# espiriki/Garbage_Classification_RCA

Hardware: AMD Instinct MI355X
Metric: train samples/sec (image+text pairs), MM-RCA ViT-B16+DistilBERT (higher is better)
Workload: dtype bf16

## Files before the change

garbage_classification_rca_amd/csrc/gemm256.hip:

```cpp
#include "common.h"
#include "lds_asm.h"
#include <type_traits>
#include <mutex>

typedef __attribute__((ext_vector_type(4))) float f32x4;
typedef __attribute__((address_space(3))) void lds_void;
typedef const __attribute__((address_space(1))) void gbl_void;

#define HT_BYTES (128 * 64 * 2)
#define STAGE_BYTES (4 * HT_BYTES)
#define LDS256_BYTES (128 * (256 * 4 + 16))
#define SLOT_A0 0
#define SLOT_A1 1
#define SLOT_B0 2
#define SLOT_B1 3

__device__ __forceinline__ int krow_f2(int row) { return (row & 3) | (((row >> 3) & 1) << 2); }

__device__ __forceinline__ void stage_half(const bf16_t* src0, const bf16_t* src1, char* lds_piece0) {
  __builtin_amdgcn_global_load_lds((gbl_void*)src0, (lds_void*)(lds_piece0), 16, 0, 0);
  __builtin_amdgcn_global_load_lds((gbl_void*)src1, (lds_void*)(lds_piece0 + 1024), 16, 0, 0);
}

template <bool F4>
// ... 400 lines not shown
    for (int a = 0; a < 2; ++a)
#pragma unroll
      for (int b = 0; b < 2; ++b)
#pragma unroll
        for (int i = 0; i < 4; ++i)
#pragma unroll
          for (int j = 0; j < 2; ++j) acc[a][b][i][j] = (f32x4){0.f, 0.f, 0.f, 0.f};
    frag_bases();
    if (wr) BARRIER();
    __builtin_amdgcn_sched_barrier(0);
    const int ntv = (X3 && !F4) ? nseg * nt : tile_nk;
    if constexpr (F4) {
      if (ti + 1 < my_tiles) {
        for (int t = 0; t < ntv; ++t) K_TILE_G4(ISSUE_P, 1, 1, 1, 1, 8, 8, 10, 8);
      } else {
        for (int t = 0; t < ntv - 2; ++t) K_TILE_G4(ISSUE_P, 1, 1, 1, 1, 8, 8, 10, 8);
        K_TILE_G4(ISSUE_P, 1, 1, 0, 0, 8, 8, 8, 4);
        K_TILE_G4(ISSUE_P, 0, 0, 0, 0, 2, 0, 0, 0);
      }
    } else
    if (ti + 1 < my_tiles) {
      for (int t = 0; t < ntv; ++t) K_TILE_G(ISSUE_P, 1, 1, 1, 1, 8, 8, 10, 8);
    } else {
      for (int t = 0; t < ntv - 2; ++t) K_TILE_G(ISSUE_P, 1, 1, 1, 1, 8, 8, 10, 8);
      K_TILE_G(ISSUE_P, 1, 1, 0, 0, 8, 8, 8, 4);
      K_TILE_G(ISSUE_P, 0, 0, 0, 0, 2, 0, 0, 0);
    }
    if (!wr) BARRIER();
    __builtin_amdgcn_sched_barrier(0);

    if constexpr (!X3 || F4) {
      if (ti >= my_dp) {
        int lane_s = lane;
        asm volatile("" : "+v"(lane_s));
        float* const mine = sk_slab + ((int64_t)(unit_tile * sk_split + unit_part) * 65536 + wave * 8192 + lane_s * 4);
#pragma unroll
        for (int f = 0; f < 32; ++f)
          asm volatile("global_store_dwordx4 %0, %1, off sc1" :: "v"(mine + f * 256), "v"(acc[f >> 4][(f >> 3) & 1][(f >> 1) & 3][f & 1]) : "memory");
        asm volatile("s_waitcnt vmcnt(0)" ::: "memory");
        __syncthreads();
        volatile unsigned* const flag = reinterpret_cast<volatile unsigned*>(smem + EP_BASE);
        if (threadIdx.x == 0) {
          const unsigned arrived = __hip_atomic_fetch_add(sk_count + unit_tile, 1u, __ATOMIC_RELAXED, __HIP_MEMORY_SCOPE_AGENT);
          if (arrived == (unsigned)sk_split - 1u)
            __hip_atomic_store(sk_count + unit_tile, 0u, __ATOMIC_RELAXED, __HIP_MEMORY_SCOPE_AGENT);
          *flag = arrived;
        }
        __syncthreads();
        const bool last = *flag == (unsigned)sk_split - 1u;
        __syncthreads();
        if (!last) break;
        asm volatile("" : "+v"(lane_s));
        const float* const all = sk_slab + ((int64_t)(unit_tile * sk_split) * 65536 + wave * 8192 + lane_s * 4);
#define SK_LD16(R, SRC)                                                                                                       \
        asm volatile("global_load_dwordx4 %0, %16, off sc1\n\tglobal_load_dwordx4 %1, %16, off offset:1024 sc1\n\t"         \
                     "global_load_dwordx4 %2, %16, off offset:2048 sc1\n\tglobal_load_dwordx4 %3, %16, off offset:3072 sc1\n\t" \
                     "global_load_dwordx4 %4, %17, off sc1\n\tglobal_load_dwordx4 %5, %17, off offset:1024 sc1\n\t"         \
                     "global_load_dwordx4 %6, %17, off offset:2048 sc1\n\tglobal_load_dwordx4 %7, %17, off offset:3072 sc1\n\t" \
                     "global_load_dwordx4 %8, %18, off sc1\n\tglobal_load_dwordx4 %9, %18, off offset:1024 sc1\n\t"         \
                     "global_load_dwordx4 %10, %18, off offset:2048 sc1\n\tglobal_load_dwordx4 %11, %18, off offset:3072 sc1\n\t" \
                     "global_load_dwordx4 %12, %19, off sc1\n\tglobal_load_dwordx4 %13, %19, off offset:1024 sc1\n\t"       \
                     "global_load_dwordx4 %14, %19, off offset:2048 sc1\n\tglobal_load_dwordx4 %15, %19, off offset:3072 sc1\n\t" \
                     "s_waitcnt vmcnt(0)"                                                                                     \
                     : "=&v"(R[0]), "=&v"(R[1]), "=&v"(R[2]), "=&v"(R[3]), "=&v"(R[4]), "=&v"(R[5]), "=&v"(R[6]), "=&v"(R[7]),     \
                       "=&v"(R[8]), "=&v"(R[9]), "=&v"(R[10]), "=&v"(R[11]), "=&v"(R[12]), "=&v"(R[13]), "=&v"(R[14]), "=&v"(R[15]) \
                     : "v"((SRC)), "v"((SRC) + 1024), "v"((SRC) + 2048), "v"((SRC) + 3072) : "memory")
        for (int part = 0; part < sk_split; ++part) {
          const float* const src = all + (int64_t)part * 65536;
#pragma unroll
          for (int h = 0; h < 2; ++h) {
            f32x4 t[16];
            SK_LD16(t, src + h * 4096);
#pragma unroll
            for (int f = 0; f < 16; ++f) {
              f32x4& c = acc[h][(f >> 3) & 1][(f >> 1) & 3][f & 1];
              c = part == 0 ? t[f] : c + t[f];
            }
          }
        }
#undef SK_LD16
      }
    }

    int lane_e = lane;
    asm volatile("" : "+v"(lane_e));
    const int e16 = lane_e & 15, eg = lane_e >> 4;
    const unsigned wbase0 = lds0 + EP_BASE + wave * 4096 + e16 * 256 + ((eg ^ (e16 & 7)) << 4);
    const unsigned rbase0 = lds0 + EP_BASE + wave * 4096 + eg * 256;
    const int64_t ncol = n_blk + 64 * wc + 4 * e16;
    const unsigned lane_off = (unsigned)(eg * (int)ldc + 4 * e16) * 2u;
    float bv[4] = {0.f, 0.f, 0.f, 0.f};
    if constexpr (act != MMRCA_ACT_MUL) {
      if (bias) {
        if constexpr (X3) {
          const f32x4 b4 = *reinterpret_cast<const f32x4*>(reinterpret_cast<const float*>(bias) + ncol);
#pragma unroll
          for (int r = 0; r < 4; ++r) bv[r] = b4[r];
        } else {
          bf16x4 b4 = *reinterpret_cast<const bf16x4*>(bias + ncol);
#pragma unroll
          for (int r = 0; r < 4; ++r) bv[r] = (float)b4[r];
        }
      }
    }
    float csum[4] = {0.f, 0.f, 0.f, 0.f};
    const bool full = m_blk + 256 <= M;
    asm volatile("s_nop 15\n\ts_nop 15" ::: "memory");
    constexpr bool SIDE = ADD || act == MMRCA_ACT_MUL;
    bf16x4 side[SIDE ? 32 : 1];
    if constexpr (SIDE) {
      const char* sp = reinterpret_cast<const char*>(ADD ? (const bf16_t*)addend : (const bf16_t*)preact);
      if (!(dbg & 2)) {
#pragma unroll
        for (int q = 0; q < 32; ++q) {
          const int64_t urow = m_blk + 128 * (q >> 4) + 64 * wr + 4 * (q & 15);
          const int64_t ub = (urow * ldc + n_blk + 64 * wc) * 2;
          side[q] = *reinterpret_cast<const bf16x4*>(sp + ub + lane_off);
        }
      }
    }
    auto passes = [&](auto ragged_tag) {
      constexpr bool RAGGED = decltype(ragged_tag)::value;
  #pragma unroll
      for (int pass = 0; pass < 8; ++pass) {
        const int a = pass >> 2, i = pass & 3;
        {
          const unsigned wbase1 = wbase0 ^ 64u;
          DS_WRITE_B128(wbase0, acc[a][0][i][0], 0);
          DS_WRITE_B128(wbase1, acc[a][0][i][1], 0);
          DS_WRITE_B128(wbase0, acc[a][1][i][0], 128);
          DS_WRITE_B128(wbase1, acc[a][1][i][1], 128);
        }
        const int64_t urow0 = m_blk + 128 * a + 64 * wr + 16 * i;
        constexpr int RB = SIDE ? 2 : 4;
  #pragma unroll
        for (int it0 = 0; it0 < 4; it0 += RB) {
          f32x4 cr[RB];
  #pragma unroll
          for (int u = 0; u < RB; ++u) {
            const int it = it0 + u;
            const unsigned rb = rbase0 + it * 1024 + ((unsigned)(e16 ^ ((4 * it + eg) & 7)) << 4);
            DS_READ_B128(cr[u], rb, 0);
          }
          if constexpr (RB == 4) asm volatile("s_waitcnt lgkmcnt(0)" : "+v"(cr[0]), "+v"(cr[1]), "+v"(cr[2]), "+v"(cr[3]) :: "memory");
          else asm volatile("s_waitcnt lgkmcnt(0)" : "+v"(cr[0]), "+v"(cr[1]) :: "memory");
  #pragma unroll
          for (int u = 0; u < RB; ++u) {
            const int it = it0 + u;
            float v[4] = {cr[u][0], cr[u][1], cr[u][2], cr[u][3]};
            if constexpr (act != MMRCA_ACT_MUL) {
  #pragma unroll
              for (int r = 0; r < 4; ++r) v[r] += bv[r];
            }
            bf16x4 po;
            [[maybe_unused]] float pf[4] = {0.f, 0.f, 0.f, 0.f};
            constexpr bool store_pre = act == MMRCA_ACT_GELU_SAVE_GRAD;
            if constexpr (act == MMRCA_ACT_MUL) {
  #pragma unroll
              for (int r = 0; r < 4; ++r) v[r] *= (float)side[4 * pass + it][r];
            } else if constexpr (act == MMRCA_ACT_GELU_SAVE_GRAD) {
              float gr[4];
              gelu_and_grad_fast4(v, gr);
  #pragma unroll
              for (int r = 0; r < 4; ++r) { po[r] = (bf16_t)gr[r]; pf[r] = gr[r]; }
            } else if constexpr (act == MMRCA_ACT_GELU) {
              gelu_fast4(v);
            }
            if constexpr (ADD) {
  #pragma unroll
              for (int r = 0; r < 4; ++r) v[r] += (float)side[4 * pass + it][r];
            }
            bf16x4 o;
  #pragma unroll
            for (int r = 0; r < 4; ++r) o[r] = (bf16_t)v[r];
            const bool ok = !RAGGED || urow0 + 4 * it + eg < M;
            if (ok) {
              if constexpr (act == MMRCA_ACT_MUL) {
  #pragma unroll
                for (int r = 0; r < 4; ++r) csum[r] += (float)o[r];
              }
              const int64_t ub = ((urow0 + 4 * it) * ldc + n_blk + 64 * wc) * 2;
              if constexpr (X3) {
                if (store_pre) {
                  if (pre16) *reinterpret_cast<bf16x4*>(reinterpret_cast<char*>(preact) + ub + lane_off) = po;
                  else *reinterpret_cast<f32x4*>(reinterpret_cast<char*>(preact) + 2 * (ub + lane_off)) = (f32x4){pf[0], pf[1], pf[2], pf[3]};
                }
                if constexpr (PLANES) {
                  bf16x4 lo;
#pragma unroll
                  for (int r = 0; r < 4; ++r) lo[r] = (bf16_t)(v[r] - (float)o[r]);
                  *reinterpret_cast<bf16x4*>(reinterpret_cast<char*>(C) + ub + lane_off) = o;
                  *reinterpret_cast<bf16x4*>(reinterpret_cast<char*>(C_lo) + ub + lane_off) = lo;
                } else {
                  *reinterpret_cast<f32x4*>(reinterpret_cast<char*>(C) + 2 * (ub + lane_off)) = (f32x4){v[0], v[1], v[2], v[3]};
                }
              } else {
              if (store_pre) *reinterpret_cast<bf16x4*>(reinterpret_cast<char*>(preact) + ub + lane_off) = po;
              *reinterpret_cast<bf16x4*>(reinterpret_cast<char*>(C) + ub + lane_off) = o;
              }
            }
          }
        }
      }
    };
    if (!(dbg & 2)) {
      if (full) passes(std::false_type{}); else passes(std::true_type{});
    }
    if constexpr (act == MMRCA_ACT_MUL) {
      if (colsum) {
#pragma unroll
        for (int r = 0; r < 4; ++r) atomicAdd(colsum + ncol + r, csum[r]);
      }
    }
    __builtin_amdgcn_sched_barrier(0);
  }
}

extern int g_mmrca_dbg;

#define SK_COUNTER_BYTES 4096
#define SK_MAX_UNITS 256
struct SkWorkspace { int device; void* stream; char* base; int64_t bytes; };
static SkWorkspace g_sk_ws[32];
static int g_sk_ws_n = 0;
static std::mutex g_sk_mutex;
extern "C" int64_t mmrca_gemm_streamk_workspace_bytes(void) { return SK_COUNTER_BYTES + (int64_t)SK_MAX_UNITS * 65536 * 4; }
extern "C" int mmrca_gemm_streamk_workspace(void* workspace, int64_t bytes, void* stream) {
  MMRCA_REQUIRE(workspace == nullptr || (bytes >= mmrca_gemm_streamk_workspace_bytes() && (((uintptr_t)workspace) & 15) == 0),
                "gemm_streamk_workspace: needs %lld bytes, 16-byte aligned, zero-filled", (long long)mmrca_gemm_streamk_workspace_bytes());
  int dev = 0;
  (void)hipGetDevice(&dev);
  std::lock_guard<std::mutex> lock(g_sk_mutex);
  for (int i = 0; i < g_sk_ws_n; ++i)
    if (g_sk_ws[i].stream == stream && g_sk_ws[i].device == dev) {
      if (workspace) { g_sk_ws[i].base = (char*)workspace; g_sk_ws[i].bytes = bytes; }
      else g_sk_ws[i] = g_sk_ws[--g_sk_ws_n];
      return 0;
    }
  if (!workspace || g_sk_ws_n == 32) return 0;
  g_sk_ws[g_sk_ws_n++] = SkWorkspace{dev, stream, (char*)workspace, bytes};
  return 0;
}
static char* sk_workspace_of(void* stream) {
  if (g_sk_ws_n == 0) return nullptr;
  int dev = 0;
  (void)hipGetDevice(&dev);
  std::lock_guard<std::mutex> lock(g_sk_mutex);
  for (int i = 0; i < g_sk_ws_n; ++i)
    if (g_sk_ws[i].stream == stream && g_sk_ws[i].device == dev) return g_sk_ws[i].base;
  return nullptr;
}
static int g_sk_max = 4, g_sk_min_ksteps = 24;
static bool g_sk_bf16 = false;
extern "C" int mmrca_gemm_streamk_config(int max_split, int min_ksteps, int bf16_products) {
  if (max_split >= 0) g_sk_max = max_split;
  if (min_ksteps >= 0) g_sk_min_ksteps = min_ksteps;
  if (bf16_products >= 0) g_sk_bf16 = bf16_products != 0;
  return 0;
}
int mmrca_gemm256_streamk_split(int64_t M, int64_t N, int64_t ksteps, void* stream, bool x3) {
  const int sk_max = g_sk_max;
  if ((!x3 && !g_sk_bf16) || ksteps < g_sk_min_ksteps || !sk_workspace_of(stream)) return 0;
  const int64_t tiles = ((M + 255) / 256) * (N / 256);
  const int ncu = cu_count();
  if (tiles < ncu) return 0;
  const int64_t left = tiles % ncu;
  if (left == 0) return 0;
  int64_t split = ncu / left;
  if (split > ksteps / 2) split = ksteps / 2;
  if (split > sk_max) split = sk_max;
  return split >= 2 ? (int)split : 0;
}
int64_t mmrca_gemm256_round_split(int64_t M, int64_t N) {
  const int64_t ncu = cu_count(), tm = M / 256, tn = N / 256, tiles = tm * tn;
  const int64_t rounds = tiles / ncu, rem = tiles - rounds * ncu;
  const int64_t m_split = rounds * ncu / tn;
  return rounds >= 1 && rem * 100 >= 25 * ncu && rem * 100 < 60 * ncu && m_split >= 1 && m_split < tm ? m_split * 256 : 0;
}
template <bool AK, bool BK2, int ACT, bool ADD, bool X3 = false, bool PLANES = false, bool F4 = false>
static void launch_p256(const void* A, const void* B, void* C, const void* bias, const void* addend, void* preact, int64_t M,
                        int64_t N, int64_t K, int64_t lda, int64_t ldb, int64_t ldc, float* colsum, hipStream_t st,
                        const void* A_lo = nullptr, const void* B_lo = nullptr, void* C_lo = nullptr, int nseg = 3, int pre16 = 0) {
  const int tiles_m = (int)((M + 255) / 256), tiles_n = (int)(N / 256);
  const int ncu = cu_count();
  int grid = tiles_m * tiles_n < ncu ? ((tiles_m * tiles_n) & ~7) : ncu;
  if (grid < 8) grid = 8;
  constexpr int LDS_P = 2 * STAGE_BYTES + 32768;
  int sk_split = 0;
  char* sk_ws = nullptr;
  if constexpr (!X3 || F4) {
    sk_split = mmrca_gemm256_streamk_split(M, N, K / (F4 ? 32 : 64), (void*)st, X3);
    if (sk_split >= 2) sk_ws = sk_workspace_of((void*)st);
    if (!sk_ws) sk_split = 0;
  }
  MMRCA_MAX_LDS(LDS_P, gemm_p256_k<AK, BK2, ACT, ADD, X3, PLANES, F4>);
  hipLaunchKernelGGL((gemm_p256_k<AK, BK2, ACT, ADD, X3, PLANES, F4>), dim3(grid), dim3(512), LDS_P, st, (const bf16_t*)A, (const bf16_t*)B,
                     (bf16_t*)C, (const bf16_t*)bias, (const bf16_t*)addend, (bf16_t*)preact, M, N, K, lda, ldb, ldc, tiles_m,
                     tiles_n, colsum, 0, g_mmrca_dbg, (const bf16_t*)A_lo,
                     (const bf16_t*)B_lo, (bf16_t*)C_lo, nseg, pre16, (float*)(sk_ws ? sk_ws + SK_COUNTER_BYTES : nullptr),
                     (unsigned*)sk_ws, sk_split);
}

int g_mmrca_dbg = 0;
extern "C" int mmrca_debug_set(int v) { g_mmrca_dbg = v; return 0; }

bool mmrca_gemm256_ok(int64_t M, int64_t N, int64_t K, int a_layout, int act, bool has_addend, bool has_preact, bool has_colsum, bool has_bias) {
  if (!(N % 256 == 0 && K % 64 == 0 && K >= 128 && a_layout == MMRCA_ROWK)) return false;
  if (act == MMRCA_ACT_NONE) return !has_preact && !has_colsum;
  if (act == MMRCA_ACT_GELU_SAVE_GRAD) return has_preact && !has_addend && !has_colsum;
  if (act == MMRCA_ACT_GELU) return !has_preact && !has_addend && !has_colsum;
  if (act == MMRCA_ACT_MUL) return has_preact && !has_addend && !has_bias;
  return false;
}

int mmrca_gemm256(const void* A, const void* B, void* C, const void* bias, const void* addend, void* preact, int64_t M,
                  int64_t N, int64_t K, int64_t lda, int64_t ldb, int64_t ldc, int a_layout, int b_layout, int act,
                  float* colsum, hipStream_t st) {
  const bool bk = b_layout == MMRCA_KROW;
  MMRCA_REQUIRE(mmrca_gemm256_ok(M, N, K, a_layout, act, addend != nullptr, preact != nullptr, colsum != nullptr, bias != nullptr),
                "gemm(mfma256): shape / epilogue combination not built");
  MMRCA_REQUIRE(M * lda * 2 < (1ll << 32) && (bk ? K * ldb : N * ldb) * 2 < (1ll << 32) && M * ldc * 2 < (1ll << 32),
                "gemm(mfma256): operands must be smaller than 4 GiB");
  with_bools([&](auto bk_) {
    const auto launch = [&](auto mode, auto add) {
      launch_p256<false, bk_, mode, add>(A, B, C, bias, addend, preact, M, N, K, lda, ldb, ldc, colsum, st);
    };
    using std::integral_constant;
    if (act == MMRCA_ACT_GELU_SAVE_GRAD) launch(integral_constant<int, MMRCA_ACT_GELU_SAVE_GRAD>{}, std::false_type{});
    else if (act == MMRCA_ACT_GELU) launch(integral_constant<int, MMRCA_ACT_GELU>{}, std::false_type{});
    else if (act == MMRCA_ACT_MUL) launch(integral_constant<int, MMRCA_ACT_MUL>{}, std::false_type{});
    else if (addend) launch(integral_constant<int, MMRCA_ACT_NONE>{}, std::true_type{});
    else launch(integral_constant<int, MMRCA_ACT_NONE>{}, std::false_type{});
  }, bk);
  MMRCA_CHECK_LAUNCH("gemm(mfma256)");
  return 0;
}


bool mmrca_gemm256_x3_ok(int64_t M, int64_t N, int64_t K, int a_layout, int act, bool has_addend, bool has_colsum) {
  if (!(N % 256 == 0 && K % 64 == 0 && K >= 128 && a_layout == MMRCA_ROWK) || has_addend || has_colsum) return false;
  return act == MMRCA_ACT_NONE || act == MMRCA_ACT_GELU_SAVE_GRAD;
}

int mmrca_gemm256_x3_streamk_split(int64_t M, int64_t N, int64_t K, int b_layout, bool has_a_lo, bool has_b_lo, void* stream) {
  if (!(b_layout != MMRCA_KROW && has_a_lo && has_b_lo && K % 32 == 0 && K >= 64)) return 0;
  return mmrca_gemm256_streamk_split(M, N, K / 32, stream, true);
}

int mmrca_gemm256_x3(const void* A_hi, const void* A_lo, const void* B_hi, const void* B_lo, void* C, void* C_lo, const void* bias,
                     void* preact, int64_t M, int64_t N, int64_t K, int64_t lda, int64_t ldb, int64_t ldc, int b_layout, int act,
                     hipStream_t st, int pre16) {
  const bool bk = b_layout == MMRCA_KROW;
  MMRCA_REQUIRE(M * lda * 2 < (1ll << 32) && (bk ? K * ldb : N * ldb) * 2 < (1ll << 32) && M * ldc * 4 < (1ll << 32),
                "gemm_x3(mfma256): operands must be smaller than 4 GiB");
  const bool gelu = act == MMRCA_ACT_GELU_SAVE_GRAD, planes = C_lo != nullptr;
  if (!bk && A_lo && B_lo && K % 32 == 0 && K >= 64) {
    with_bools([&](auto gelu_, auto planes_) {
      launch_p256<false, false, gelu_ ? MMRCA_ACT_GELU_SAVE_GRAD : MMRCA_ACT_NONE, false, true, planes_, true>(
          A_hi, B_hi, C, bias, nullptr, preact, M, N, K, lda, ldb, ldc, nullptr, st, A_lo, B_lo, C_lo, 3, pre16);
    }, gelu, planes);
    MMRCA_CHECK_LAUNCH("gemm_x3(mfma256,fused)");
    return 0;
  }
  with_bools([&](auto bk_, auto gelu_, auto planes_) {
    launch_p256<false, bk_, gelu_ ? MMRCA_ACT_GELU_SAVE_GRAD : MMRCA_ACT_NONE, false, true, planes_>(
        A_hi, B_hi, C, bias, nullptr, preact, M, N, K, lda, ldb, ldc, nullptr, st, A_lo, B_lo, C_lo, A_lo ? (B_lo ? 3 : 2) : 1, pre16);
  }, bk, gelu, planes);
  MMRCA_CHECK_LAUNCH("gemm_x3(mfma256)");
  return 0;
}

__global__ void __launch_bounds__(256)
splitk_reduce256_k(const float* __restrict__ slab, float* __restrict__ C, int64_t ldc, int ntiles, int tiles_n, int splits, int64_t M, int64_t N) {
  const int tile = blockIdx.x >> 6;
  const int idx = ((blockIdx.x & 63) << 8) + threadIdx.x;
  const float* src = slab + (int64_t)tile * 65536 + (int64_t)idx * 4;
  f32x4 s = *reinterpret_cast<const f32x4*>(src);
  for (int k = 1; k < splits; ++k) {
    const f32x4 v = *reinterpret_cast<const f32x4*>(src + (int64_t)k * ntiles * 65536);
    s += v;
  }
  const int w = idx >> 11, f = (idx >> 6) & 31, lane = idx & 63;
  const int a = f >> 4, b = (f >> 3) & 1, i = (f >> 1) & 3, j = f & 1;
  const int wr = w >> 2, wc = w & 3, l16 = lane & 15, g = lane >> 4;
  const int row = 128 * a + 64 * wr + 16 * i + l16, col = 128 * b + 32 * wc + 16 * j + 4 * g;
  const int tm = tile / tiles_n, tn = tile % tiles_n;
  if ((int64_t)tm * 256 + row >= M || (int64_t)tn * 256 + col >= N) return;
  float* dst = C + ((int64_t)tm * 256 + row) * ldc + (int64_t)tn * 256 + col;
  f32x4 c = *reinterpret_cast<f32x4*>(dst);
  c += s;
  *reinterpret_cast<f32x4*>(dst) = c;
}

extern "C" int64_t mmrca_gemm_splitk_workspace_bytes(int64_t M, int64_t N) {
  if (M <= 0 || N <= 0 || M % 8 || N % 8) return 0;
  const int64_t tiles = ((M + 255) / 256) * ((N + 255) / 256);
  if (tiles > 256) return 0;
  return (256 / tiles) * tiles * 65536 * 4;
}

static int gemm_splitk_impl(const void* A, const void* A_lo, const void* B, const void* B_lo, float* C, void* workspace,
                           int64_t workspace_bytes, int64_t M, int64_t N, int64_t K, int64_t lda, int64_t ldb, int64_t ldc,
                           int a_layout, int b_layout, void* stream) {
  const bool x3 = A_lo != nullptr;
  const int nseg = x3 ? (B_lo ? 3 : 2) : 1;
  MMRCA_REQUIRE(A && B && C && workspace, "gemm_splitk: null operand");
  const bool ragged = M % 256 != 0 || N % 256 != 0;
  MMRCA_REQUIRE(M > 0 && N > 0 && M % 8 == 0 && N % 8 == 0 && K >= 128 && K % 64 == 0 &&
                (!ragged || (a_layout == MMRCA_KROW && b_layout == MMRCA_KROW && !A_lo)),
                "gemm_splitk: needs K %% 64 == 0, K >= 128 and M, N multiples of 256 (K-major bf16 operands: of 8) (got M=%lld N=%lld K=%lld)",
                (long long)M, (long long)N, (long long)K);
  MMRCA_REQUIRE(lda % 8 == 0 && ldb % 8 == 0 && ldc % 4 == 0 && (((uintptr_t)A | (uintptr_t)B | (uintptr_t)C | (uintptr_t)workspace) & 15) == 0,
                "gemm_splitk: operands must be 16-byte aligned");
  MMRCA_REQUIRE(lda >= (a_layout == MMRCA_ROWK ? K : M) && ldb >= (b_layout == MMRCA_ROWK ? K : N) && ldc >= N, "gemm_splitk: leading dimension too small");
  const int tiles_m = (int)((M + 255) / 256), tiles_n = (int)((N + 255) / 256), tiles = tiles_m * tiles_n;
  MMRCA_REQUIRE(tiles <= 256, "gemm_splitk: more than 256 output tiles (use mmrca_gemm)");
  const int64_t ksteps = (int64_t)nseg * (K / 64);
  int64_t splits64 = 256 / tiles;
  if (splits64 > ksteps / 2) splits64 = ksteps / 2;
  const int splits = (int)splits64;
  const int ksteps_base = (int)(ksteps / splits), ksteps_rem = (int)(ksteps % splits);
  MMRCA_REQUIRE(workspace_bytes >= (int64_t)splits * tiles * 65536 * 4, "gemm_splitk: workspace too small (%lld < %lld bytes)",
                (long long)workspace_bytes, (long long)splits * tiles * 65536 * 4);
  hipStream_t st = (hipStream_t)stream;
  const bool ak = a_layout == MMRCA_KROW, bk = b_layout == MMRCA_KROW;
#define LSLAB(AK_, BK_, X3_)                                                                                                     \
  do {                                                                                                                           \
    MMRCA_MAX_LDS(LDS256_BYTES, gemm_mfma256_k<AK_, BK_, MODE_SLAB, X3_>); \
    hipLaunchKernelGGL((gemm_mfma256_k<AK_, BK_, MODE_SLAB, X3_>), dim3((tiles * splits + 7) / 8 * 8), dim3(512), LDS256_BYTES, st, (const bf16_t*)A,      \
                       (const bf16_t*)B, (bf16_t*)nullptr, (const bf16_t*)nullptr, (const bf16_t*)nullptr, (bf16_t*)nullptr, M, N, K, \
                       lda, ldb, ldc, tiles_m, tiles_n, ksteps_base, ksteps_rem, (float*)workspace, (float*)nullptr, splits,    \
                       (const bf16_t*)A_lo, (const bf16_t*)B_lo, nseg);                                                         \
  } while (0)
  if (x3) {
    if (!ak && !bk) LSLAB(false, false, true);
    else if (!ak && bk) LSLAB(false, true, true);
    else if (ak && !bk) LSLAB(true, false, true);
    else LSLAB(true, true, true);
  } else {
    if (!ak && !bk) LSLAB(false, false, false);
    else if (!ak && bk) LSLAB(false, true, false);
    else if (ak && !bk) LSLAB(true, false, false);
    else LSLAB(true, true, false);
  }
#undef LSLAB
  MMRCA_CHECK_LAUNCH("gemm_splitk(mfma256)");
  hipLaunchKernelGGL(splitk_reduce256_k, dim3(tiles * 64), dim3(256), 0, st, (const float*)workspace, C, ldc, tiles, tiles_n, splits, M, N);
  MMRCA_CHECK_LAUNCH("gemm_splitk(reduce)");
  return 0;
}

extern "C" int mmrca_gemm_splitk(const void* A, const void* B, float* C, void* workspace, int64_t workspace_bytes, int64_t M,
                                 int64_t N, int64_t K, int64_t lda, int64_t ldb, int64_t ldc, int a_layout, int b_layout,
                                 void* stream) {
  return gemm_splitk_impl(A, nullptr, B, nullptr, C, workspace, workspace_bytes, M, N, K, lda, ldb, ldc, a_layout, b_layout, stream);
}

extern "C" int mmrca_gemm_splitk_x3(const void* A_hi, const void* A_lo, const void* B_hi, const void* B_lo, float* C, void* workspace,
                                    int64_t workspace_bytes, int64_t M, int64_t N, int64_t K, int64_t lda, int64_t ldb, int64_t ldc,
                                    int a_layout, int b_layout, void* stream) {
  MMRCA_REQUIRE(A_lo || !B_lo, "gemm_x3(splitk): a B lo plane without an A lo plane is not a supported pass set");
  return gemm_splitk_impl(A_hi, A_lo, B_hi, B_lo, C, workspace, workspace_bytes, M, N, K, lda, ldb, ldc, a_layout, b_layout, stream);
}
```

garbage_classification_rca_amd/lib.py:

```python
from __future__ import annotations

import ctypes as C
import os
import subprocess
from types import SimpleNamespace
from typing import Optional

import torch

from . import abi

_HERE = os.path.dirname(os.path.abspath(__file__))
LIB_PATH = os.path.join(_HERE, "libmmrca.so")

F32, BF16 = 0, 1
ACT_NONE, ACT_GELU, ACT_GELU_BWD, ACT_GELU_SAVE_GRAD, ACT_MUL, ACT_GELU_SAVE_GRAD_BF16 = 0, 1, 2, 3, 4, 5
ROWK, KROW = 0, 1
IMPL_AUTO, IMPL_REF, IMPL_MFMA, IMPL_MFMA256, IMPL_MFMA_PERSIST, IMPL_MFMA_BK32, IMPL_MFMA_1STAGE, IMPL_MFMA_TALL, IMPL_MFMA_256W, IMPL_MFMA_256X4 = 0, 1, 2, 3, 4, 5, 6, 7, 8, 9

HEAD_FIELDS = [f"{blk}_{leaf}" for blk in ("sai", "sat", "c1", "c2")
               for leaf in ("wq", "bq", "wk", "bk", "wv", "bv", "g", "b")] + ["fin_w", "fin_b"]


class HeadPtrs(C.Structure):
    _fields_ = [(n, C.c_void_p) for n in HEAD_FIELDS]


class MmrcaError(RuntimeError):
    pass


def build_library(force: bool = False) -> str:
    src_dir = os.path.join(_HERE, "csrc")
    cmd = ["make", "-C", src_dir, "-j8"]
    if force:
        subprocess.run(["make", "-C", src_dir, "clean"], check=True, capture_output=True)
    r = subprocess.run(cmd, capture_output=True, text=True)
    if r.returncode != 0 or not os.path.exists(LIB_PATH) or not os.path.exists(os.path.join(_HERE, "libmmrca_jpeg.so")):
        raise MmrcaError("building libmmrca.so / libmmrca_jpeg.so failed:\n" + r.stdout[-4000:] + r.stderr[-4000:])
    return LIB_PATH


_lib = None
_protos = None


def _prototypes():
    global _protos
    if _protos is None:
        head = C.POINTER(HeadPtrs)
        try:
            _protos = abi.prototypes(struct_pointers={"MmrcaHeadWeights": head, "MmrcaHeadGrads": head})
        except abi.MmrcaError as e:
            raise MmrcaError(str(e)) from None
    return _protos


def load(build_if_missing: bool = False):
    global _lib
    if _lib is not None:
        return _lib
    if not os.path.exists(LIB_PATH):
        if build_if_missing:
            build_library()
        else:
            raise MmrcaError(f"{LIB_PATH} not found: the HIP extension is required (run __graft_entry__.build()); "
                             "there is no CPU fallback")
    lib = C.CDLL(LIB_PATH)
    try:
        abi.bind(lib, _prototypes())
    except abi.MmrcaError as e:
        raise MmrcaError(str(e)) from None
    _lib = lib
    return lib


def _check(rc: int, what: str):
    if rc != 0:
        raise MmrcaError(f"{what} failed ({rc}): {load().mmrca_last_error().decode()}")


def dtype_code(dt: torch.dtype) -> int:
    if dt == torch.float32:
        return F32
    if dt == torch.bfloat16:
        return BF16
    raise MmrcaError(f"unsupported dtype {dt}")


def ptr(t: Optional[torch.Tensor]):
    return None if t is None else t.data_ptr()


_raw_stream = getattr(torch._C, "_cuda_getCurrentRawStream", None)
_cur_device = getattr(torch._C, "_cuda_getDevice", None)


def stream_ptr() -> int:
    if _raw_stream is not None and _cur_device is not None:
        return _raw_stream(_cur_device())
    return torch.cuda.current_stream().cuda_stream


def _dev(t: torch.Tensor, name: str):
    if not t.is_cuda:
        raise MmrcaError(f"{name}: tensor must live in HBM (got device {t.device}); the product path has no CPU fallback")


def _launch(name, *args):
    rc = getattr(_lib if _lib is not None else load(), name)(*args, stream_ptr())
    if rc != 0:
        _check(rc, name)


GEMM_PROFILE = None
KERNEL_PROFILE = None


def _events():
    e0, e1 = torch.cuda.Event(enable_timing=True), torch.cuda.Event(enable_timing=True)
    e0.record()
    return e0, e1


class _Bracket:

    def __init__(self, kind, meta):
        self.kind, self.meta, self.on = kind, meta, KERNEL_PROFILE is not None

    def __enter__(self):
        if self.on:
            self.e0, self.e1 = _events()
        return self

    def __exit__(self, *exc):
        if self.on and exc[0] is None:
            self.e1.record()
            KERNEL_PROFILE.append((self.kind, self.meta, self.e0, self.e1))
        return False


def _esz(dt):
    return 2 if dt == BF16 else 4


GEMM_SHAPES = None
CONV_PROFILE = None


_STREAMK_WS = {}
STREAMK = os.environ.get("MMRCA_SK", "1") != "0"


def streamk_workspace(M, N, device, force=False):
    if not (STREAMK or force) or N % 256 or ((M + 255) // 256) * (N // 256) < 256:
        return
    st = stream_ptr()
    key = (device.index if device.index is not None else torch.cuda.current_device(), st)
    if key in _STREAMK_WS:
        return
    if not force and torch.cuda.is_current_stream_capturing():
        return
    need = int(load().mmrca_gemm_streamk_workspace_bytes())
    ws = torch.zeros(need, dtype=torch.uint8, device=device)
    _launch("mmrca_gemm_streamk_workspace", ptr(ws), need)
    _STREAMK_WS[key] = ws


def gemm_is_mfma(M, N, K, a_layout, dtype, impl):
    return dtype == BF16 and impl != IMPL_REF and N % 128 == 0 and K % 64 == 0 and (a_layout == ROWK or M % 128 == 0)


def gemm(A, B, Cout, *, bias=None, addend=None, preact=None, M, N, K, lda, ldb, ldc, a_layout=ROWK, b_layout=ROWK,
         act=ACT_NONE, accum=False, dtype, impl=IMPL_AUTO, colsum=None, rows_readable=None):
    _dev(A, "gemm A")
    if rows_readable is not None:
        if accum:
            raise MmrcaError("gemm: rows_readable is not available in accumulate mode")
        _launch("mmrca_gemm_rows", ptr(A), ptr(B), ptr(Cout), ptr(bias), ptr(addend), ptr(preact), ptr(colsum), M, N, K, lda, ldb, ldc,
                int(rows_readable[0]), int(rows_readable[1]), a_layout, b_layout, act, dtype, impl)
        return
    prof = GEMM_PROFILE is not None and (gemm_is_mfma(M, N, K, a_layout, dtype, impl) or (dtype == F32 and impl != IMPL_REF))
    timed = prof or CONV_PROFILE is not None
    if timed:
        e0, e1 = _events()
    if colsum is not None:
        if accum:
            raise MmrcaError("gemm: colsum is not available in accumulate mode")
        _launch("mmrca_gemm_colsum", ptr(A), ptr(B), ptr(Cout), ptr(bias), ptr(addend), ptr(preact), ptr(colsum), M, N, K, lda, ldb, ldc, a_layout,
                b_layout, act, dtype, impl)
    else:
        _launch("mmrca_gemm", ptr(A), ptr(B), ptr(Cout), ptr(bias), ptr(addend), ptr(preact), M, N, K, lda, ldb, ldc, a_layout, b_layout, act,
                int(accum), dtype, impl)
    if timed:
        e1.record()
    if prof:
        GEMM_PROFILE.append((2.0 * M * N * K, (a_layout, b_layout, int(accum)), e0, e1, (M, N, K, act)))
    if CONV_PROFILE is not None:
        es = _esz(dtype)
        side = (1 if addend is not None else 0) + (1 if preact is not None else 0)
        nbytes = int((M * K + N * K) * es + M * N * ((4 if accum else es) + side * es))
        CONV_PROFILE.append(("GEMM (1x1 conv / patch matrix / text encoder)", nbytes, e0, e1))
        if GEMM_SHAPES is not None:
            GEMM_SHAPES.append((M, N, K, a_layout, b_layout, int(accum), nbytes, e0, e1))


SPLITK_WS_BYTES = 64 << 20


def gemm_splitk_ok(M, N, K, dtype):
    return dtype == BF16 and M % 256 == 0 and N % 256 == 0 and K % 64 == 0 and K >= 128 and (M // 256) * (N // 256) <= 256


def gemm_splitk_ragged_ok(M, N, K, dtype):
    return (dtype == BF16 and M % 8 == 0 and N % 8 == 0 and K % 64 == 0 and K >= 128
            and ((M + 255) // 256) * ((N + 255) // 256) <= 256)


def gemm_splitk(A, B, Cout, workspace, *, M, N, K, lda, ldb, ldc, a_layout=KROW, b_layout=KROW):
    _dev(A, "gemm_splitk A")
    prof = GEMM_PROFILE is not None
    if prof:
        e0, e1 = _events()
    _launch("mmrca_gemm_splitk", ptr(A), ptr(B), ptr(Cout), ptr(workspace), workspace.numel() * workspace.element_size(), M, N, K, lda, ldb, ldc,
            a_layout, b_layout)
    if prof:
        e1.record()
        GEMM_PROFILE.append((2.0 * M * N * K, (a_layout, b_layout, 1), e0, e1, (M, N, K, ACT_NONE)))
    if CONV_PROFILE is not None:
        CONV_PROFILE.append(("GEMM (1x1 conv / patch matrix / text encoder)", int((M * K + N * K) * 2 + M * N * 4), None, None))


def gemm_x3(A, B, Cout, *, C_lo=None, bias=None, addend=None, preact=None, colsum=None, M, N, K, lda, ldb, ldc, a_layout=ROWK,
            b_layout=ROWK, act=ACT_NONE, accum=False, impl=IMPL_AUTO):
    _dev(A[0], "gemm_x3 A")
    if not accum:
        streamk_workspace(M, N, A[0].device)
    prof = GEMM_PROFILE is not None
    if prof:
        e0, e1 = _events()
    _launch("mmrca_gemm_x3", ptr(A[0]), ptr(A[1]), ptr(B[0]), ptr(B[1]), ptr(Cout), ptr(C_lo), ptr(bias), ptr(addend), ptr(preact), ptr(colsum), M, N,
            K, lda, ldb, ldc, a_layout, b_layout, act, int(accum), impl)
    if prof:
        e1.record()
        GEMM_PROFILE.append((6.0 * M * N * K, (a_layout, b_layout, int(accum)), e0, e1, (M, N, K, act)))


def gemm_splitk_x3(A, B, Cout, workspace, *, M, N, K, lda, ldb, ldc, a_layout=KROW, b_layout=KROW):
    _dev(A[0], "gemm_splitk_x3 A")
    prof = GEMM_PROFILE is not None
    if prof:
        e0, e1 = _events()
    _launch("mmrca_gemm_splitk_x3", ptr(A[0]), ptr(A[1]), ptr(B[0]), ptr(B[1]), ptr(Cout), ptr(workspace),
            workspace.numel() * workspace.element_size(), M, N, K, lda, ldb, ldc, a_layout, b_layout)
    if prof:
        e1.record()
        GEMM_PROFILE.append((6.0 * M * N * K, (a_layout, b_layout, 1), e0, e1, (M, N, K, ACT_NONE)))


def split_f32(src, hi, lo, n):
    _dev(src, "split src")
    _launch("mmrca_split_f32", ptr(src), ptr(hi), ptr(lo), n)


def colsum_accum(dY, db, M, N, ld, dtype):
    _launch("mmrca_colsum_accum", ptr(dY), ptr(db), M, N, ld, dtype)


def gelu_bwd(dG, H, dH, n, dtype):
    _launch("mmrca_gelu_bwd", ptr(dG), ptr(H), ptr(dH), n, dtype)


def gelu_bwd_colsum(dG, H, dH, db, M, N, ld, dtype):
    _launch("mmrca_gelu_bwd_colsum", ptr(dG), ptr(H), ptr(dH), ptr(db), M, N, ld, dtype)


def mha_fwd(qkv, key_mask, out, lse, B, H, S, dh, scale, dtype, impl=IMPL_AUTO, drop_p=0.0, drop_seed=0, cu=None):
    _dev(qkv, "mha qkv")
    with _Bracket("mha_fwd", (B, H, S, dh, cu is not None)):
        _launch("mmrca_mha_fwd", ptr(qkv), ptr(key_mask), ptr(out), ptr(lse), B, H, S, dh, scale, drop_p, drop_seed, ptr(cu), dtype, impl)


def mha_fwd_planes_ok(S, dh):
    return dh == 64 and 1 <= S <= 208


def mha_fwd_planes(qkv, key_mask, out, out_planes, lse, B, H, S, dh, scale, drop_p=0.0, drop_seed=0, cu=None):
    _dev(qkv, "mha qkv")
    with _Bracket("mha_fwd", (B, H, S, dh, cu is not None)):
        _launch("mmrca_mha_fwd_planes", ptr(qkv), ptr(key_mask), ptr(out), ptr(out_planes[0]), ptr(out_planes[1]), ptr(lse), B, H, S, dh, scale,
                drop_p, drop_seed, ptr(cu))


def mha_fwd_planes_in(qkv_planes, key_mask, out, out_planes, lse, B, H, S, dh, scale, drop_p=0.0, drop_seed=0, cu=None):
    _dev(qkv_planes[0], "mha qkv")
    with _Bracket("mha_fwd", (B, H, S, dh, cu is not None)):
        _launch("mmrca_mha_fwd_planes_in", ptr(qkv_planes[0]), ptr(qkv_planes[1]), ptr(key_mask), ptr(out), ptr(out_planes[0]), ptr(out_planes[1]),
                ptr(lse), B, H, S, dh, scale, drop_p, drop_seed, ptr(cu))


def mha_fwd_x3_ok(S, dh):
    return dh == 64 and 1 <= S <= 512


def mha_fwd_x3(qkv_planes, key_mask, out_planes, lse, B, H, S, dh, scale, drop_p=0.0, drop_seed=0, cu=None):
    _dev(qkv_planes[0], "mha qkv")
    with _Bracket("mha_fwd", (B, H, S, dh, cu is not None)):
        _launch("mmrca_mha_fwd_x3", ptr(qkv_planes[0]), ptr(qkv_planes[1]), ptr(key_mask), ptr(out_planes[0]), ptr(out_planes[1]), ptr(lse), B, H, S,
                dh, scale, drop_p, drop_seed, ptr(cu))


def mha_bwd(qkv, key_mask, out, dout, lse, dqkv, B, H, S, dh, scale, dtype, impl=IMPL_AUTO, drop_p=0.0, drop_seed=0, colsum=None,
            cu=None, rows=None):
    with _Bracket("mha_bwd", (B, H, S, dh, cu is not None)):
        if colsum is not None:
            _launch("mmrca_mha_bwd_colsum", ptr(qkv), ptr(key_mask), ptr(out), ptr(dout), ptr(lse), ptr(dqkv), ptr(colsum),
                    B * S if rows is None else rows, B, H, S, dh, scale, drop_p, drop_seed, ptr(cu), dtype, impl)
            return
        _launch("mmrca_mha_bwd", ptr(qkv), ptr(key_mask), ptr(out), ptr(dout), ptr(lse), ptr(dqkv), B, H, S, dh, scale, drop_p, drop_seed, ptr(cu),
                dtype, impl)


def mha_cross_fwd(q, ldq, k, ldk, v, ldv, out, ldo, B, H, Sq, Skv, dh, scale, dtype, impl=IMPL_AUTO, drop_p=0.0, drop_seed=0):
    _dev(q, "q"); _dev(k, "k"); _dev(v, "v"); _dev(out, "out")
    _launch("mmrca_mha_cross_fwd", ptr(q), ldq, ptr(k), ldk, ptr(v), ldv, ptr(out), ldo, B, H, Sq, Skv, dh, scale, drop_p, drop_seed, dtype, impl)


def mha_cross_fwd_x3(q, ldq, k, ldk, v, ldv, out_planes, ldo, B, H, Sq, Skv, dh, scale, drop_p=0.0, drop_seed=0):
    _dev(q, "q"); _dev(k, "k"); _dev(v, "v"); _dev(out_planes[0], "out")
    if q.dtype != torch.float32 or k.dtype != torch.float32 or v.dtype != torch.float32 or out_planes[0].dtype != torch.bfloat16:
        raise MmrcaError("mha_cross_fwd_x3: q / k / v must be fp32 and the output planes bf16")
    _launch("mmrca_mha_cross_fwd_x3", ptr(q), ldq, ptr(k), ldk, ptr(v), ldv, ptr(out_planes[0]), ptr(out_planes[1]), ldo, B, H, Sq, Skv, dh, scale,
            drop_p, drop_seed)


def mha_cls_fwd(qkv, key_mask, out, lse, B, H, S, dh, scale, dtype, drop_p=0.0, drop_seed=0, cu=None):
    _dev(qkv, "mha_cls qkv")
    _launch("mmrca_mha_cls_fwd", ptr(qkv), ptr(key_mask), ptr(out), ptr(lse), B, H, S, dh, scale, drop_p, drop_seed, ptr(cu), dtype)


def mha_cls_bwd(qkv, key_mask, out, dout, lse, dqkv, B, H, S, dh, scale, dtype, drop_p=0.0, drop_seed=0, cu=None):
    _launch("mmrca_mha_cls_bwd", ptr(qkv), ptr(key_mask), ptr(out), ptr(dout), ptr(lse), ptr(dqkv), B, H, S, dh, scale, drop_p, drop_seed, ptr(cu),
            dtype)


def add_layernorm_fwd(x, res, gamma, beta, sum_out, y, mean, rstd, rows, D, ld_x, ld_y, eps, dtype,
                      in_drop=(0.0, 0), out_drop=(0.0, 0), y_planes=None):
    _dev(x, "layernorm x")
    if y_planes is not None:
        _launch("mmrca_add_layernorm_fwd_x3", ptr(x), ptr(res), ptr(gamma), ptr(beta), ptr(sum_out), ptr(y), ptr(y_planes[0]), ptr(y_planes[1]),
                ptr(mean), ptr(rstd), rows, D, ld_x, ld_y, eps, in_drop[0], in_drop[1], out_drop[0], out_drop[1])
        return
    _launch("mmrca_add_layernorm_fwd", ptr(x), ptr(res), ptr(gamma), ptr(beta), ptr(sum_out), ptr(y), ptr(mean), ptr(rstd), rows, D, ld_x, ld_y, eps,
            in_drop[0], in_drop[1], out_drop[0], out_drop[1], dtype)


def layernorm_bwd(dy, s, gamma, mean, rstd, dres, ds, dgamma, dbeta, rows, D, ld_dy, ld_s, ld_ds, dtype,
                  dy_drop=(0.0, 0), branch_drop=(0.0, 0), dbranch=None, dcol=None, dcol_branch=None):
    _launch("mmrca_layernorm_bwd", ptr(dy), ptr(s), ptr(gamma), ptr(mean), ptr(rstd), ptr(dres), ptr(ds), ptr(dgamma), ptr(dbeta), rows, D, ld_dy,
            ld_s, ld_ds, dy_drop[0], dy_drop[1], branch_drop[0], branch_drop[1], ptr(dbranch), ptr(dcol), ptr(dcol_branch), dtype)


def layernorm_bwd_mixed(dy, s, gamma, mean, rstd, dres, ds, dgamma, dbeta, rows, D, ld_dy, ld_s, ld_ds,
                        dy_drop=(0.0, 0), branch_drop=(0.0, 0), dbranch=None, dcol=None, dcol_branch=None):
    _launch("mmrca_layernorm_bwd_mixed", ptr(dy), ptr(s), ptr(gamma), ptr(mean), ptr(rstd), ptr(dres), ptr(ds), ptr(dgamma), ptr(dbeta), rows, D,
            ld_dy, ld_s, ld_ds, dy_drop[0], dy_drop[1], branch_drop[0], branch_drop[1], ptr(dbranch), ptr(dcol), ptr(dcol_branch))


def embed_fwd(ids, pos_ids, word, pos, type_row, out, rows, D, dtype):
    _dev(ids, "embed ids")
    _launch("mmrca_embed_fwd", ptr(ids), ptr(pos_ids), ptr(word), ptr(pos), ptr(type_row), ptr(out), rows, D, dtype)


def embed_bwd(dout, ids, pos_ids, dword, dpos, dtype_row, rows, D, dtype, pad_id=-1, pos_pad_id=-1):
    _launch("mmrca_embed_bwd", ptr(dout), ptr(ids), ptr(pos_ids), ptr(dword), ptr(dpos), ptr(dtype_row), rows, D, pad_id, pos_pad_id, dtype)


def patchify_fwd(images, patches, B, Cc, Himg, Wimg, P, dtype):
    _dev(images, "patchify images")
    _launch("mmrca_patchify_fwd", ptr(images), ptr(patches), B, Cc, Himg, Wimg, P, dtype)


def vit_assemble_fwd(proj, cls, pos, x, B, nP, D, dtype):
    _launch("mmrca_vit_assemble_fwd", ptr(proj), ptr(cls), ptr(pos), ptr(x), B, nP, D, dtype)


def vit_assemble_bwd(dx, dproj, dcls, dpos, B, nP, D, dtype):
    _launch("mmrca_vit_assemble_bwd", ptr(dx), ptr(dproj), ptr(dcls), ptr(dpos), B, nP, D, dtype)


def head_fwd(img, txt, w: HeadPtrs, logits, B, d_img, d_txt, n_classes, reverse, mode, drop_p, seed, dtype):
    _dev(img, "head img")
    with _Bracket("head_fwd", (B, d_img, d_txt)):
        _launch("mmrca_head_fwd", ptr(img), ptr(txt), C.byref(w), ptr(logits), B, d_img, d_txt, n_classes, int(reverse), mode, drop_p, seed, dtype)


_HEAD_WS = {}


def head_bwd_workspace_bytes(B, d_img, d_txt) -> int:
    return int(load().mmrca_head_bwd_workspace_bytes(B, d_img, d_txt))


def head_bwd(dlogits, img, txt, w: HeadPtrs, g: HeadPtrs, dimg, dtxt, B, d_img, d_txt, n_classes, reverse, mode, drop_p, seed, dtype,
             workspace=None):
    need = head_bwd_workspace_bytes(B, d_img, d_txt)
    if workspace is None:
        key = (img.device.index, stream_ptr())
        workspace = _HEAD_WS.get(key)
        if workspace is None or workspace.numel() < need:
            workspace = _HEAD_WS[key] = torch.empty(need, dtype=torch.uint8, device=img.device)
    with _Bracket("head_bwd", (B, d_img, d_txt)):
        _launch("mmrca_head_bwd", ptr(dlogits), ptr(img), ptr(txt), C.byref(w), C.byref(g), ptr(dimg), ptr(dtxt), B, d_img, d_txt, n_classes,
                int(reverse), mode, drop_p, seed, dtype, ptr(workspace), workspace.numel() * workspace.element_size())


def linear_cls_fwd(feat, ld, W, b, logits, B, F, Cc, drop_p, seed, dtype):
    _dev(feat, "linear_cls feat")
    with _Bracket("linear_cls_fwd", (B, F, Cc)):
        _launch("mmrca_linear_cls_fwd", ptr(feat), ld, ptr(W), ptr(b), ptr(logits), B, F, Cc, float(drop_p), int(seed) & 0xFFFFFFFFFFFFFFFF, dtype)


def linear_cls_bwd(dlogits, feat, ld, W, dW, db, dfeat, B, F, Cc, drop_p, seed, dtype):
    _dev(dlogits, "linear_cls dlogits")
    with _Bracket("linear_cls_bwd", (B, F, Cc)):
        _launch("mmrca_linear_cls_bwd", ptr(dlogits), ptr(feat), ld, ptr(W), ptr(dW), ptr(db), ptr(dfeat), B, F, Cc, float(drop_p),
                int(seed) & 0xFFFFFFFFFFFFFFFF, dtype)


def xent_fwd_bwd(logits, labels, class_w, smoothing, loss, dlogits, B, Cc, grad_scale=1.0):
    _dev(logits, "xent logits")
    _launch("mmrca_xent_fwd_bwd", ptr(logits), ptr(labels), ptr(class_w), smoothing, ptr(loss), ptr(dlogits), B, Cc, grad_scale)


def sgd_step(p, g, lp, n, lr, wd, grad_scale=1.0, lp_lo=None):
    _dev(p, "sgd params")
    if lp_lo is not None:
        _launch("mmrca_sgd_step_x3", ptr(p), ptr(g), ptr(lp), ptr(lp_lo), n, lr, wd, grad_scale)
        return
    _launch("mmrca_sgd_step", ptr(p), ptr(g), ptr(lp), n, lr, wd, grad_scale)


def adamw_step(p, g, m, v, lp, n, lr, b1, b2, eps, wd, step, grad_scale=1.0, lp_lo=None):
    _dev(p, "adamw params")
    if lp_lo is not None:
        _launch("mmrca_adamw_step_x3", ptr(p), ptr(g), ptr(m), ptr(v), ptr(lp), ptr(lp_lo), n, lr, b1, b2, eps, wd, step, grad_scale)
        return
    _launch("mmrca_adamw_step", ptr(p), ptr(g), ptr(m), ptr(v), ptr(lp), n, lr, b1, b2, eps, wd, step, grad_scale)


SEED_EPOCH_STRIDE = 1000003
def _u64v(seed):
    return int(seed) & 0xFFFFFFFFFFFFFFFF


def hier_pool_fwd(x, out, ld_out, B, H, W, Cc, k, dtype):
    _dev(x, "hier_pool x")
    with _Bracket("hier_pool_fwd", (B, H, W, Cc, k)):
        _launch("mmrca_hier_pool_fwd", ptr(x), ptr(out), ld_out, B, H, W, Cc, k, dtype)


def hier_pool_bwd(d, ld_d, dx, B, H, W, Cc, k, dtype):
    _dev(dx, "hier_pool dx")
    with _Bracket("hier_pool_bwd", (B, H, W, Cc, k)):
        _launch("mmrca_hier_pool_bwd", ptr(d), ld_d, ptr(dx), B, H, W, Cc, k, dtype)


def _seg_array(seg_off):
    return (C.c_int * len(seg_off))(*[int(v) for v in seg_off])


def hier_norm_fwd(raw, x, inv, B, ld, seg_off, nseg_a, drop_p, seed_a, seed_b):
    _dev(raw, "hier_norm raw")
    with _Bracket("hier_norm_fwd", (B, ld)):
        _launch("mmrca_hier_norm_fwd", ptr(raw), ptr(x), ptr(inv), B, ld, _seg_array(seg_off), len(seg_off) - 1, nseg_a, float(drop_p), _u64v(seed_a),
                _u64v(seed_b))


def hier_norm_bwd(dx, raw, inv, draw, B, ld, seg_off, nseg_a, drop_p, seed_a, seed_b):
    _dev(dx, "hier_norm dx")
    with _Bracket("hier_norm_bwd", (B, ld)):
        _launch("mmrca_hier_norm_bwd", ptr(dx), ptr(raw), ptr(inv), ptr(draw), B, ld, _seg_array(seg_off), len(seg_off) - 1, nseg_a, float(drop_p),
                _u64v(seed_a), _u64v(seed_b))


def hier_linear_workspace_bytes(B, N, K) -> int:
    return int(load().mmrca_hier_linear_workspace_bytes(B, N, K))


def hier_linear_relu_fwd(X, ldx, W, b, Y, ldy, ws, B, N, K):
    _dev(X, "hier_linear X")
    with _Bracket("hier_linear_relu_fwd", (B, N, K)):
        _launch("mmrca_hier_linear_relu_fwd", ptr(X), ldx, ptr(W), ptr(b), ptr(Y), ldy, ptr(ws), ws.numel() * ws.element_size(), B, N, K)


def hier_linear_relu_bwd(dY, lddy, Y, ldy, X, ldx, W, dW, db, dX, lddx, ws, B, N, K):
    _dev(dY, "hier_linear dY")
    with _Bracket("hier_linear_relu_bwd", (B, N, K)):
        _launch("mmrca_hier_linear_relu_bwd", ptr(dY), lddy, ptr(Y), ldy, ptr(X), ldx, ptr(W), ptr(dW), ptr(db), ptr(dX), lddx, ptr(ws),
                0 if ws is None else ws.numel() * ws.element_size(), B, N, K)


def gru_linear_fwd(X, ldx, W, b, Y, ldy, B, N, K, relu=False):
    _dev(X, "gru_linear X")
    with _Bracket("gru_linear_fwd", (B, N, K)):
        _launch("mmrca_gru_linear_fwd", ptr(X), ldx, ptr(W), ptr(b), ptr(Y), ldy, B, N, K, int(bool(relu)))


def gru_linear_bwd(dY, lddy, Y, ldy, X, ldx, W, dW, db, dX, lddx, B, N, K):
    _dev(dY, "gru_linear dY")
# ... 385 lines not shown
```

Measured before the change: 7028.

## Add a 4-wave 256x256 split-K slab kernel for KROW×KROW long-K GEMMs

Adds a new split-K slab kernel that computes a 256x256 tile with 4 waves (each owning a 128x128 sub-tile with an 8x8 MFMA accumulator array) instead of 8 waves, plus a matching reduce layout. It is chosen automatically for non-x3 KROW/KROW split-K GEMMs when each split has at least 16 k-steps, and a debug-flag bit field can force either loop. The aim is higher per-wave data reuse and fewer LDS reads per MFMA on weight-gradient style GEMMs. The trade-off is heavy accumulator register pressure and lower occupancy.

```diff
diff --git a/garbage_classification_rca_amd/csrc/gemm256.hip b/garbage_classification_rca_amd/csrc/gemm256.hip
--- a/garbage_classification_rca_amd/csrc/gemm256.hip
+++ b/garbage_classification_rca_amd/csrc/gemm256.hip
@@ -726,7 +726,8 @@
 }
 
 int g_mmrca_dbg = 0;
-extern "C" int mmrca_debug_set(int v) { g_mmrca_dbg = v; return 0; }
+static int g_splitk_loop = 0;
+extern "C" int mmrca_debug_set(int v) { g_mmrca_dbg = v & 0x0fffffff; g_splitk_loop = (v >> 28) & 3; return 0; }
 
 bool mmrca_gemm256_ok(int64_t M, int64_t N, int64_t K, int a_layout, int act, bool has_addend, bool has_preact, bool has_colsum, bool has_bias) {
   if (!(N % 256 == 0 && K % 64 == 0 && K >= 128 && a_layout == MMRCA_ROWK)) return false;
@@ -795,6 +796,125 @@
 }
 
 __global__ void __launch_bounds__(256)
+gemm_slab4w_k(const bf16_t* __restrict__ A, const bf16_t* __restrict__ B, int64_t M, int64_t N, int64_t lda, int64_t ldb, int tiles_m,
+              int tiles_n, int ksteps_base, int ksteps_rem, float* __restrict__ slab, int splits) {
+  extern __shared__ __attribute__((aligned(16))) char smem[];
+  const int wave = __builtin_amdgcn_readfirstlane(threadIdx.x >> 6), lane = threadIdx.x & 63;
+  const int wr = wave >> 1, wc = wave & 1;
+
+  const int nwg = tiles_m * tiles_n;
+  const int total = nwg * splits;
+  const int per_xcd = (total + 7) >> 3;
+  const int idx = ((int)blockIdx.x & 7) * per_xcd + ((int)blockIdx.x >> 3);
+  if (((int)blockIdx.x >> 3) >= per_xcd || idx >= total) return;
+  const int yb = idx / nwg, wgid = idx - yb * nwg;
+  const int tm = wgid / tiles_n, tn = wgid - tm * tiles_n;
+  const int64_t m_blk = (int64_t)tm * 256, n_blk = (int64_t)tn * 256;
+  const int64_t kbeg = 64 * ((int64_t)yb * ksteps_base + (yb < ksteps_rem ? yb : ksteps_rem));
+  const int nt = ksteps_base + (yb < ksteps_rem ? 1 : 0);
+
+  f32x4 acc[8][8];
+#pragma unroll
+  for (int i = 0; i < 8; ++i)
+#pragma unroll
+    for (int j = 0; j < 8; ++j) acc[i][j] = (f32x4){0.f, 0.f, 0.f, 0.f};
+
+  unsigned oa[2][2], ob[2][2];
+#pragma unroll
+  for (int h = 0; h < 2; ++h)
+#pragma unroll
+    for (int ii = 0; ii < 2; ++ii) {
+      oa[h][ii] = (unsigned)((piece_src<true>(A, lda, m_blk + 128 * h, M, wave * 2 + ii, lane) - A + kbeg * lda) * 2);
+      ob[h][ii] = (unsigned)((piece_src<true>(B, ldb, n_blk + 128 * h, N, wave * 2 + ii, lane) - B + kbeg * ldb) * 2);
+    }
+  const unsigned a_step = (unsigned)(64 * lda), b_step = (unsigned)(64 * ldb);
+  char* const my_piece = smem + wave * 2048;
+  int issue_stage = 0;
+#define SRC4(P, off) reinterpret_cast<const bf16_t*>(reinterpret_cast<const char*>(P) + (off))
+#define ISSUE4_HALF(KS, which)                                                                                                   \
+  do {                                                                                                                           \
+    char* const d_ = my_piece + issue_stage + (KS) * 8192;                                                                       \
+    if ((which) == 0) { stage_half(SRC4(A, oa[0][0]), SRC4(A, oa[0][1]), d_ + SLOT_A0 * HT_BYTES); oa[0][0] += a_step; oa[0][1] += a_step; } \
+    else if ((which) == 1) { stage_half(SRC4(A, oa[1][0]), SRC4(A, oa[1][1]), d_ + SLOT_A1 * HT_BYTES); oa[1][0] += a_step; oa[1][1] += a_step; } \
+    else if ((which) == 2) { stage_half(SRC4(B, ob[0][0]), SRC4(B, ob[0][1]), d_ + SLOT_B0 * HT_BYTES); ob[0][0] += b_step; ob[0][1] += b_step; } \
+    else { stage_half(SRC4(B, ob[1][0]), SRC4(B, ob[1][1]), d_ + SLOT_B1 * HT_BYTES); ob[1][0] += b_step; ob[1][1] += b_step;    \
+           if (KS) issue_stage ^= STAGE_BYTES; }                                                                                 \
+  } while (0)
+
+  const unsigned lds0 = (unsigned)(uintptr_t)(lds_void*)smem;
+  const int g = lane >> 4, l16 = lane & 15;
+  unsigned abase[8], bbase[8];
+  {
+    const int q = l16 >> 2, p = l16 & 3, row = 8 * g + q;
+#pragma unroll
+    for (int f = 0; f < 8; ++f) {
+      abase[f] = lds0 + (SLOT_A0 + wr) * HT_BYTES + row * 256 + ((f ^ krow_f2(row)) << 5) + p * 8;
+      bbase[f] = lds0 + (SLOT_B0 + wc) * HT_BYTES + row * 256 + ((f ^ krow_f2(row)) << 5) + p * 8;
+    }
+  }
+  Frag<true> fa[2][4][2], fb[2][4][2];
+#define READ4(S, KS, f)                                                                                                          \
+  do {                                                                                                                           \
+    if ((f) < 8) read_frag<true, (KS) * 8192>(fa[S][((f) & 7) >> 1][(f) & 1], abase[(f) & 7]);                                   \
+    else read_frag<true, (KS) * 8192>(fb[S][((f) & 7) >> 1][(f) & 1], bbase[(f) & 7]);                                           \
+  } while (0)
+#define TOGGLE4()                                                                                                                \
+  do {                                                                                                                           \
+    _Pragma("unroll") for (int x = 0; x < 8; ++x) { abase[x] ^= STAGE_BYTES; bbase[x] ^= STAGE_BYTES; }                          \
+  } while (0)
+#define MFMA4(ACC, BV, AV) asm volatile("v_mfma_f32_16x16x32_bf16 %0, %1, %2, %0" : "+a"(ACC) : "v"(BV), "v"(AV))
+#define STEP4(S, RD, RKS, ISS, WAIT, W)                                                                                          \
+  do {                                                                                                                           \
+    lgkm0(fa[S]); lgkm0(fb[S]);                                                                                                  \
+    if (WAIT) { VMCNT(W); BARRIER(); }                                                                                           \
+    bf16x8 av_[8], bv_[8];                                                                                                       \
+    _Pragma("unroll") for (int f = 0; f < 8; ++f) { av_[f] = frag_val(fa[S][f >> 1][f & 1]); bv_[f] = frag_val(fb[S][f >> 1][f & 1]); } \
+    _Pragma("unroll") for (int q4 = 0; q4 < 16; ++q4) {                                                                          \
+      _Pragma("unroll") for (int m = 4 * q4; m < 4 * q4 + 4; ++m) MFMA4(acc[m >> 3][m & 7], bv_[m & 7], av_[m >> 3]);            \
+      if (RD) READ4((S) ^ 1, RKS, q4);                                                                                           \
+      if (ISS) { if (q4 == 1) ISSUE4_HALF(S, 0); else if (q4 == 5) ISSUE4_HALF(S, 2); else if (q4 == 9) ISSUE4_HALF(S, 1);       \
+                 else if (q4 == 13) ISSUE4_HALF(S, 3); }                                                                         \
+    }                                                                                                                            \
+  } while (0)
+
+  ISSUE4_HALF(0, 0); ISSUE4_HALF(0, 1); ISSUE4_HALF(0, 2); ISSUE4_HALF(0, 3);
+  ISSUE4_HALF(1, 0); ISSUE4_HALF(1, 1); ISSUE4_HALF(1, 2); ISSUE4_HALF(1, 3);
+  ISSUE4_HALF(0, 0); ISSUE4_HALF(0, 1); ISSUE4_HALF(0, 2); ISSUE4_HALF(0, 3);
+  ISSUE4_HALF(1, 0); ISSUE4_HALF(1, 1); ISSUE4_HALF(1, 2); ISSUE4_HALF(1, 3);
+  VMCNT(24);
+  BARRIER();
+  __builtin_amdgcn_sched_barrier(0);
+#pragma unroll
+  for (int f = 0; f < 16; ++f) READ4(0, 0, f);
+  __builtin_amdgcn_sched_barrier(0);
+
+  for (int t = 0; t < nt - 2; ++t) {
+    STEP4(0, 1, 1, 1, 1, 16);
+    TOGGLE4();
+    STEP4(1, 1, 0, 1, 1, 16);
+  }
+  STEP4(0, 1, 1, 0, 1, 16);
+  TOGGLE4();
+  STEP4(1, 1, 0, 0, 1, 8);
+  STEP4(0, 1, 1, 0, 1, 0);
+  STEP4(1, 0, 0, 0, 0, 0);
+  asm volatile("s_nop 15\n\ts_nop 15" ::: "memory");
+
+  float* dst = slab + ((int64_t)yb * nwg + (int64_t)tm * tiles_n + tn) * 65536 + wave * 16384 + lane * 4;
+#pragma unroll
+  for (int i = 0; i < 8; ++i)
+#pragma unroll
+    for (int j = 0; j < 8; ++j) *reinterpret_cast<f32x4*>(dst + (i * 8 + j) * 256) = acc[i][j];
+#undef STEP4
+#undef MFMA4
+#undef TOGGLE4
+#undef READ4
+#undef ISSUE4_HALF
+#undef SRC4
+}
+
+template <bool W4>
+__global__ void __launch_bounds__(256)
 splitk_reduce256_k(const float* __restrict__ slab, float* __restrict__ C, int64_t ldc, int ntiles, int tiles_n, int splits, int64_t M, int64_t N) {
   const int tile = blockIdx.x >> 6;
   const int idx = ((blockIdx.x & 63) << 8) + threadIdx.x;
@@ -804,10 +924,17 @@
     const f32x4 v = *reinterpret_cast<const f32x4*>(src + (int64_t)k * ntiles * 65536);
     s += v;
   }
-  const int w = idx >> 11, f = (idx >> 6) & 31, lane = idx & 63;
-  const int a = f >> 4, b = (f >> 3) & 1, i = (f >> 1) & 3, j = f & 1;
-  const int wr = w >> 2, wc = w & 3, l16 = lane & 15, g = lane >> 4;
-  const int row = 128 * a + 64 * wr + 16 * i + l16, col = 128 * b + 32 * wc + 16 * j + 4 * g;
+  const int lane = idx & 63, l16 = lane & 15, g = lane >> 4;
+  int row, col;
+  if constexpr (W4) {
+    const int w = idx >> 12, f = (idx >> 6) & 63;
+    row = 128 * (w >> 1) + 16 * (f >> 3) + l16, col = 128 * (w & 1) + 16 * (f & 7) + 4 * g;
+  } else {
+    const int w = idx >> 11, f = (idx >> 6) & 31;
+    const int a = f >> 4, b = (f >> 3) & 1, i = (f >> 1) & 3, j = f & 1;
+    const int wr = w >> 2, wc = w & 3;
+    row = 128 * a + 64 * wr + 16 * i + l16, col = 128 * b + 32 * wc + 16 * j + 4 * g;
+  }
   const int tm = tile / tiles_n, tn = tile % tiles_n;
   if ((int64_t)tm * 256 + row >= M || (int64_t)tn * 256 + col >= N) return;
   float* dst = C + ((int64_t)tm * 256 + row) * ldc + (int64_t)tn * 256 + col;
@@ -856,7 +983,14 @@
                        lda, ldb, ldc, tiles_m, tiles_n, ksteps_base, ksteps_rem, (float*)workspace, (float*)nullptr, splits,    \
                        (const bf16_t*)A_lo, (const bf16_t*)B_lo, nseg);                                                         \
   } while (0)
-  if (x3) {
+  const int loop_sel = g_splitk_loop;
+  const bool w4 = !x3 && ak && bk && K * lda * 2 < (1ll << 32) && K * ldb * 2 < (1ll << 32) &&
+                  (loop_sel == 2 || (loop_sel == 0 && ksteps_base >= 16));
+  if (w4) {
+    MMRCA_MAX_LDS(2 * STAGE_BYTES, gemm_slab4w_k);
+    hipLaunchKernelGGL(gemm_slab4w_k, dim3((tiles * splits + 7) / 8 * 8), dim3(256), 2 * STAGE_BYTES, st, (const bf16_t*)A, (const bf16_t*)B,
+                       M, N, lda, ldb, tiles_m, tiles_n, ksteps_base, ksteps_rem, (float*)workspace, splits);
+  } else if (x3) {
     if (!ak && !bk) LSLAB(false, false, true);
     else if (!ak && bk) LSLAB(false, true, true);
     else if (ak && !bk) LSLAB(true, false, true);
@@ -869,7 +1003,8 @@
   }
 #undef LSLAB
   MMRCA_CHECK_LAUNCH("gemm_splitk(mfma256)");
-  hipLaunchKernelGGL(splitk_reduce256_k, dim3(tiles * 64), dim3(256), 0, st, (const float*)workspace, C, ldc, tiles, tiles_n, splits, M, N);
+  if (w4) hipLaunchKernelGGL(splitk_reduce256_k<true>, dim3(tiles * 64), dim3(256), 0, st, (const float*)workspace, C, ldc, tiles, tiles_n, splits, M, N);
+  else hipLaunchKernelGGL(splitk_reduce256_k<false>, dim3(tiles * 64), dim3(256), 0, st, (const float*)workspace, C, ldc, tiles, tiles_n, splits, M, N);
   MMRCA_CHECK_LAUNCH("gemm_splitk(reduce)");
   return 0;
 }
diff --git a/garbage_classification_rca_amd/lib.py b/garbage_classification_rca_amd/lib.py
--- a/garbage_classification_rca_amd/lib.py
+++ b/garbage_classification_rca_amd/lib.py
@@ -206,6 +206,7 @@
 
 
 SPLITK_WS_BYTES = 64 << 20
+SPLITK_LOOP_AUTO, SPLITK_LOOP_8W, SPLITK_LOOP_4W = 0, 1 << 28, 2 << 28
 
 
 def gemm_splitk_ok(M, N, K, dtype):
```

After: 7096 (median of 6 runs). Within noise of the previous version (+1.0%).
